# WindowsXp-Beta/nos

Measured on AMD Instinct MI355X. Metric: aggregate GPU util % + schedulable fractional pods/node at 1/2/4/8 MI355X, higher is better.
Workload: dtype fp32

## Files before the change

csrc/hip/gemm_f32h.hip:

```cpp
#include <stdlib.h>

#include <type_traits>

#include "attn_d64_planes.h"
#include "common.h"
#include "epilogue.h"
#include "lds_pipe.h"
#include "split_f16.h"

namespace {

using nos::gelu_erf;
using nos::glds16;
using nos::wait_stages;

template <int E>
using EpiC = std::integral_constant<int, E>;

struct Batch {
  int nb = 1;
  long long a = 0, rinv = 0, w = 0, csc = 0, c = 0, r = 0, bias = 0;
};

constexpr int BK = 32;

__device__ __forceinline__ int swz(int row) { return (row >> 2) & 3; }

using nos::kvp::KvOut;

struct PlaneOut {
  unsigned short* p = nullptr;
  long long pplane = 0;
  int ldp = 0;
  float sc = 1.f;
};

struct LnIo {
  const float* x = nullptr;
  const float2* sin = nullptr;
  float2* sout = nullptr;
  int ldx = 0, nparts = 0, pw = 0, spart = 0;
  float eps = 0.f, sc = 1.f;
};

__device__ __forceinline__ void chan_merge(float& n, float& mean, float& m2, float nb, float mb, float m2b) {
  const float tot = n + nb;
  if (!(nb > 0.f)) return;
  const float d = mb - mean, f = nb / tot;
  mean = fmaf(d, f, mean);
  m2 += m2b + d * d * n * f;
  n = tot;
}

template <int BM, int BN, int WGM, int WGN, bool PERSIST, int RS = 2, int MODE = 0, bool BATCHED = false>
__global__ __launch_bounds__(64 * WGM * WGN, 2) void gemm_h3_kernel(
    const _Float16* __restrict__ Ap, int lda, long long aplane, const float* __restrict__ rinv, float rconst,
    const _Float16* __restrict__ Wp, int ldw, long long wplane, const float* __restrict__ csc,
    const float* __restrict__ bias, const float* __restrict__ R, int ldr0, float* __restrict__ C, int ldc0, int M,
    int N, int K, int epi, int tiles_m, int tiles_n, KvOut kv, PlaneOut po, Batch bt, LnIo ln) {
  constexpr int NW = WGM * WGN, MI = BM / (32 * WGM), NI = BN / (32 * WGN);
  static_assert(NW == 4 && MI >= 1 && NI >= 1, "4 waves");
  constexpr int ROWB = BK * 2, CH = ROWB / 16, RPP = 1024 / ROWB;
  static_assert(RS == 2 || RS == 3, "ring depth");
  constexpr int TA = 2 * BM * ROWB, STAGE = TA + 2 * BN * ROWB;
  constexpr int APW = TA / 1024 / NW, WPW = 2 * BN * ROWB / 1024 / NW;
  static_assert(APW * NW * 1024 == TA && WPW * NW * 1024 == 2 * BN * ROWB, "equal DMA count per wave");
  constexpr int LPS = APW + WPW;
  static_assert((RS - 2) * LPS < 64, "vmcnt range");
  static_assert(MODE == 0 || (BM == 128 && !BATCHED && (BN == 128 || BN == 64) && (RS == 2 || (MODE == 2 && RS == 3))),
                "the LayerNorm hand-off runs 128 x 128 or 128 x 64 tiles (the producer also on a 3-deep ring)");
  static_assert(MODE != 2 || BM * BN * 4 <= RS * STAGE, "the statistics tile fits the ring");
  extern __shared__ __attribute__((aligned(16))) unsigned char smem[];

  const int tid = threadIdx.x, wid = __builtin_amdgcn_readfirstlane(tid >> 6), lane = tid & 63;
  const int c0 = lane & 31, h0 = lane >> 5;
  const int wm = wid / WGN, wn = wid % WGN;
  const bool wide = (epi & EPI_WIDE) != 0;
  epi &= ~EPI_WIDE;
  const int ntiles1 = tiles_m * tiles_n, ntiles = BATCHED ? ntiles1 * bt.nb : ntiles1;
  const int nk = K / BK;
  nos::XcdChunk chunk;
  if constexpr (PERSIST) {
    chunk = nos::xcd_chunk(blockIdx.x, gridDim.x, ntiles);
  } else {
    chunk.first = nos::xcd_remap(blockIdx.x, ntiles);
    chunk.end = chunk.first + 1;
    chunk.step = 1;
  }
  for (int tt = chunk.first; tt < chunk.end; tt += chunk.step) {
    if (PERSIST && tt != chunk.first) __syncthreads();
    const int bb = BATCHED ? tt / ntiles1 : 0, t1 = BATCHED ? tt - bb * ntiles1 : tt;
    const int tm = t1 / tiles_n, tn = t1 - tm * tiles_n;
    const int m0 = tm * BM, n0 = tn * BN;
    const _Float16* __restrict__ Ab = BATCHED ? Ap + bb * bt.a : Ap;
    const _Float16* __restrict__ Wb = BATCHED ? Wp + bb * bt.w : Wp;
    const float* __restrict__ rinvb = BATCHED && rinv != nullptr ? rinv + bb * bt.rinv : rinv;
    const float* __restrict__ cscb = BATCHED ? csc + bb * bt.csc : csc;
    float* __restrict__ Cb = BATCHED && C != nullptr ? C + bb * bt.c : C;
// ... 9 lines not shown
        int g = m0 + row;
        g = g < M ? g : M - 1;
        glds16(Ab + plane * aplane + (long long)g * lda + k0 + (((lane % CH) ^ swz(row)) << 3),
               dst + plane * BM * ROWB + rb * ROWB);
      }
    };
    auto stage_w = [&](int k0, unsigned char* dst) {
#pragma unroll
      for (int i = 0; i < WPW; ++i) {
        const int p = wid * WPW + i;
        const int plane = p / (BN / RPP), rb = (p % (BN / RPP)) * RPP;
        const int row = rb + lane / CH;
        int g = n0 + row;
        g = g < N ? g : N - 1;
        glds16(Wb + plane * wplane + (long long)g * ldw + k0 + (((lane % CH) ^ swz(row)) << 3),
               dst + TA + plane * BN * ROWB + rb * ROWB);
      }
    };
    auto stage = [&](int k0, unsigned char* dst) {
      stage_a(k0, dst);
      stage_w(k0, dst);
    };

    f32x16_t acc[MI][NI];
#pragma unroll
    for (int i = 0; i < MI; ++i)
#pragma unroll
      for (int j = 0; j < NI; ++j)
#pragma unroll
        for (int r = 0; r < 16; ++r) acc[i][j][r] = 0.f;

    struct Frag {
      f16x8_t a[MI][2], w[NI][2];
    };
    auto load = [&](const unsigned char* base, int s, Frag& f) {
#pragma unroll
      for (int i = 0; i < MI; ++i) {
        const int row = wm * (BM / WGM) + i * 32 + c0;
#pragma unroll
        for (int p = 0; p < 2; ++p)
          f.a[i][p] = *reinterpret_cast<const f16x8_t*>(base + p * BM * ROWB + row * ROWB +
                                                        (((2 * s + h0) ^ swz(row)) << 4));
      }
#pragma unroll
      for (int j = 0; j < NI; ++j) {
        const int row = wn * (BN / WGN) + j * 32 + c0;
#pragma unroll
        for (int p = 0; p < 2; ++p)
          f.w[j][p] = *reinterpret_cast<const f16x8_t*>(base + TA + p * BN * ROWB + row * ROWB +
                                                        (((2 * s + h0) ^ swz(row)) << 4));
      }
    };
    auto mma = [&](const Frag& f) {
#pragma unroll
      for (int i = 0; i < MI; ++i)
#pragma unroll
        for (int j = 0; j < NI; ++j) acc[i][j] = nos::mma3h(f.a[i], f.w[j], acc[i][j]);
    };

    if constexpr (MODE == 1) {
    constexpr int AR = BM * 4 / (64 * NW);
    constexpr int RSTEP = 64 * NW / 4;
    const int q = tid & 3;
    float mul[AR], add[AR];
    const float* xr[AR];
#pragma unroll
    for (int i = 0; i < AR; ++i) {
      int g = m0 + (tid >> 2) + RSTEP * i;
      g = g < M ? g : M - 1;
      xr[i] = ln.x + (long long)g * ln.ldx + q * 8;
      const float2* st = ln.sin + (long long)g * ln.nparts;
      float n = 0.f, mean = 0.f, m2 = 0.f;
      for (int p = 0; p < ln.nparts; ++p) {
        const float2 v = st[p];
        const int nb = min(ln.pw, K - p * ln.pw);
        chan_merge(n, mean, m2, (float)nb, v.x, v.y);
      }
      mul[i] = rsqrtf(m2 / (float)K + ln.eps) * ln.sc;
      add[i] = -mean * mul[i];
    }
    float4 xa[AR][2];
// ... 9 lines not shown
      for (int i = 0; i < AR; ++i) {
        const int row = (tid >> 2) + RSTEP * i;
        const float4 u = xa[i][0], w = xa[i][1];
        f16x2_t h0, l0, h1, l1, h2, l2, h3, l3;
        nos::split2h(f32x2_t{fmaf(u.x, mul[i], add[i]), fmaf(u.y, mul[i], add[i])}, h0, l0);
        nos::split2h(f32x2_t{fmaf(u.z, mul[i], add[i]), fmaf(u.w, mul[i], add[i])}, h1, l1);
        nos::split2h(f32x2_t{fmaf(w.x, mul[i], add[i]), fmaf(w.y, mul[i], add[i])}, h2, l2);
        nos::split2h(f32x2_t{fmaf(w.z, mul[i], add[i]), fmaf(w.w, mul[i], add[i])}, h3, l3);
        const int off = row * ROWB + ((q ^ swz(row)) << 4);
        *reinterpret_cast<f16x8_t*>(dst + off) = f16x8_t{h0.x, h0.y, h1.x, h1.y, h2.x, h2.y, h3.x, h3.y};
        *reinterpret_cast<f16x8_t*>(dst + BM * ROWB + off) = f16x8_t{l0.x, l0.y, l1.x, l1.y, l2.x, l2.y, l3.x, l3.y};
      }
    };
    aload(0);
    stage_w(0, smem);
    asm volatile("s_waitcnt vmcnt(0)" ::: "memory");
    awrite(smem);
    if (nk > 1) {
      aload(BK);
      stage_w(BK, smem + STAGE);
    }
    asm volatile("s_waitcnt lgkmcnt(0)" ::: "memory");
    __builtin_amdgcn_s_barrier();
    Frag fa, fb;
    load(smem, 0, fa);
    for (int kt = 0; kt < nk; ++kt) {
      const unsigned char* cur = smem + (kt & 1) * STAGE;
      load(cur, 1, fb);
      mma(fa);
      __builtin_amdgcn_sched_barrier(0);
      if (kt + 1 < nk) {
        asm volatile("s_waitcnt vmcnt(0)" ::: "memory");
        awrite(smem + ((kt + 1) & 1) * STAGE);
      }
      __builtin_amdgcn_sched_barrier(0);
      mma(fb);
      __builtin_amdgcn_sched_barrier(0);
      if (kt + 1 < nk) {
        asm volatile("s_waitcnt lgkmcnt(0)" ::: "memory");
        __builtin_amdgcn_s_barrier();
        if (kt + 2 < nk) {
          aload((kt + 2) * BK);
          stage_w((kt + 2) * BK, smem + (kt & 1) * STAGE);
        }
        load(smem + ((kt + 1) & 1) * STAGE, 0, fa);
      }
      __builtin_amdgcn_sched_barrier(0);
    }
    } else if constexpr (RS == 2) {
    stage(0, smem);
    if (nk > 1) stage(BK, smem + STAGE);
    if (nk > 1) {
      asm volatile("s_waitcnt vmcnt(%0)" ::"n"(LPS) : "memory");
    } else {
      asm volatile("s_waitcnt vmcnt(0)" ::: "memory");
    }
    __builtin_amdgcn_s_barrier();
    Frag fa, fb;
    load(smem, 0, fa);
    for (int kt = 0; kt < nk; ++kt) {
      const unsigned char* cur = smem + (kt & 1) * STAGE;
      load(cur, 1, fb);
      mma(fa);
      __builtin_amdgcn_sched_barrier(0);
      if (kt + 1 < nk) {
        asm volatile("s_waitcnt vmcnt(0)" ::: "memory");
        asm volatile("s_waitcnt lgkmcnt(0)" ::: "memory");
        __builtin_amdgcn_s_barrier();
        if (kt + 2 < nk) stage((kt + 2) * BK, smem + (kt & 1) * STAGE);
        load(smem + ((kt + 1) & 1) * STAGE, 0, fa);
      }
      mma(fb);
      __builtin_amdgcn_sched_barrier(0);
    }
    } else {
#pragma unroll
    for (int q = 0; q < RS - 1; ++q)
      if (q < nk) stage(q * BK, smem + q * STAGE);
    for (int kt = 0; kt < nk; ++kt) {
      wait_stages<LPS>(min(RS - 2, nk - 1 - kt));
      asm volatile("s_waitcnt lgkmcnt(0)" ::: "memory");
      __builtin_amdgcn_s_barrier();
      if (kt + RS - 1 < nk) stage((kt + RS - 1) * BK, smem + ((kt + RS - 1) % RS) * STAGE);
      const unsigned char* cur = smem + (kt % RS) * STAGE;
      Frag f0, f1;
      load(cur, 0, f0);
      load(cur, 1, f1);
      mma(f0);
      mma(f1);
    }
    }
    __syncthreads();

    int c = c0, h = h0, ldc = ldc0, ldr = ldr0;
    asm volatile("" : "+v"(c), "+v"(h));
    asm volatile("" : "+s"(ldc), "+s"(ldr));
    float rsv[MI][16], rbv[MI][16];
    if (rinvb != nullptr) {
#pragma unroll
      for (int i = 0; i < MI; ++i)
#pragma unroll
        for (int r = 0; r < 16; ++r) {
          const int m = m0 + wm * (BM / WGM) + i * 32 + (r & 3) + 8 * (r >> 2) + 4 * h;
          rsv[i][r] = rinvb[m < M ? m : M - 1];
        }
    } else {
#pragma unroll
      for (int i = 0; i < MI; ++i)
#pragma unroll
        for (int r = 0; r < 16; ++r) rsv[i][r] = rconst;
    }
#pragma unroll
    for (int i = 0; i < MI; ++i)
#pragma unroll
      for (int r = 0; r < 16; ++r) {
        const int m = m0 + wm * (BM / WGM) + i * 32 + (r & 3) + 8 * (r >> 2) + 4 * h;
        rbv[i][r] = (BATCHED && (epi & EPI_BIAS_ROW)) ? biasb[m < M ? m : M - 1] : 0.f;
      }
    auto epilogue = [&](auto ec) -> bool {
      constexpr int E = decltype(ec)::value;
      auto has = [&](int f) -> bool {
        if constexpr (E < 0) return (epi & f) != 0;
        else return (E & f) != 0;
      };
      if constexpr (MODE == 2) {
        float* const T = reinterpret_cast<float*>(smem);
  #pragma unroll
        for (int j = 0; j < NI; ++j) {
          const int cl = wn * (BN / WGN) + j * 32 + c;
          const int nc = n0 + cl < N ? n0 + cl : N - 1;
          const float cs = cscb[nc];
          const float p2 = has(EPI_BIAS) ? biasb[nc] : 0.f;
  #pragma unroll
          for (int i = 0; i < MI; ++i) {
  #pragma unroll
            for (int r = 0; r < 16; ++r) {
              const int rl = wm * (BM / WGM) + i * 32 + (r & 3) + 8 * (r >> 2) + 4 * h;
              float v = fmaf(acc[i][j][r], rsv[i][r] * cs, p2);
              if (has(EPI_GELU)) v = gelu_erf(v);
              if (has(EPI_RELU)) v = fmaxf(v, 0.f);
              T[rl * BN + cl] = v;
            }
          }
        }
        __syncthreads();
        const int rr = tid >> 1, hf = tid & 1, m = m0 + rr;
        const int nv = m < M ? max(0, min(BN / 2, N - n0 - hf * (BN / 2))) : 0;
        const float* tr = T + rr * BN + hf * (BN / 2);
        const long long col0 = n0 + hf * (BN / 2);
        constexpr int HV = BN / 8;
        float4 v[HV];
        const bool want = ln.sout != nullptr;
        float sum = 0.f;
        auto pass1 = [&](auto wholec) {
          constexpr bool W = decltype(wholec)::value;
  #pragma unroll
          for (int u = 0; u < HV; ++u) {
            const int k = ((u + tid) & (HV - 1)) * 4;
            v[u] = *reinterpret_cast<const float4*>(tr + k);
            if (W || k < nv) {
// ... 33 lines not shown
      }
      const bool full = m0 + BM <= M && n0 + BN <= N;
      if (full && !(has(EPI_RESID) || has(EPI_RESID_PRE)) &&
          (po.p != nullptr || (kv.kvs != nullptr && kv.S == M && n0 >= kv.qcols && kv.hd % BN == 0))) {
        unsigned short* hi;
        long long lo_off;
        int ld;
        int t = 0;
        if (po.p != nullptr) {
          hi = po.p + (long long)m0 * po.ldp + n0;
          lo_off = po.pplane;
          ld = po.ldp;
        } else {
          t = (n0 - kv.qcols) >= kv.hd;
          hi = kv.kvs + ((long long)m0 * nos::kvp::H3 + nos::kvp::H3 / 2 * t) * kv.hd + (n0 - kv.qcols - t * kv.hd);
          lo_off = kv.hd;
          ld = nos::kvp::H3 * kv.hd;
        }
        constexpr bool WIDE_FITS = 4 * BM * BN <= RS * STAGE && !BATCHED && (BN == 128 || BN == 64);
        constexpr int SWM = BN / 8 - 1;
        unsigned short* const T = reinterpret_cast<unsigned short*>(smem);
  #pragma unroll
        for (int j = 0; j < NI; ++j) {
          const int cl = wn * (BN / WGN) + j * 32 + c;
          const float cs = cscb[n0 + cl];
          const float p2 = has(EPI_BIAS) ? biasb[n0 + cl] : 0.f;
          const float osc = po.p != nullptr ? po.sc : kv.kvsc[t * (kv.hd >> 6) + ((n0 - kv.qcols - t * kv.hd + cl) >> 6)];
  #pragma unroll
          for (int i = 0; i < MI; ++i) {
  #pragma unroll
            for (int r = 0; r < 16; ++r) {
              const int rl = wm * (BM / WGM) + i * 32 + (r & 3) + 8 * (r >> 2) + 4 * h;
              float v = fmaf(acc[i][j][r], rsv[i][r] * cs, p2 + rbv[i][r]);
              if (has(EPI_GELU)) v = gelu_erf(v);
              if (has(EPI_RELU)) v = fmaxf(v, 0.f);
              const float x = v * osc;
              const _Float16 h0 = (_Float16)x;
              const _Float16 h1 = (_Float16)(x - (float)h0);
              if (WIDE_FITS && wide) {
                const int sl = rl * BN + ((((cl >> 3) ^ (rl & SWM)) << 3) | (cl & 7));
                T[sl] = __builtin_bit_cast(unsigned short, h0);
                T[BM * BN + sl] = __builtin_bit_cast(unsigned short, h1);
              } else {
                const unsigned off = (unsigned)(rl * ld + cl);
                hi[off] = __builtin_bit_cast(unsigned short, h0);
                hi[lo_off + off] = __builtin_bit_cast(unsigned short, h1);
              }
            }
          }
        }
        if (WIDE_FITS && wide) {
          __syncthreads();
          constexpr int CPR = BN / 8;
          constexpr int NCH = 2 * BM * CPR;
  #pragma unroll
          for (int q = 0; q < NCH / (64 * NW); ++q) {
            const int id = tid + q * 64 * NW;
            const int pl = id / (BM * CPR), rem = id - pl * (BM * CPR);
            const int row = rem / CPR, ch = rem - row * CPR;
            const uint4 v = *reinterpret_cast<const uint4*>(T + pl * BM * BN + row * BN + ((ch ^ (row & SWM)) << 3));
            *reinterpret_cast<uint4*>(hi + pl * lo_off + (long long)row * ld + ch * 8) = v;
          }
        }
        return true;
      }
      const bool interior = full && po.p == nullptr && (kv.kvs == nullptr || n0 + BN <= kv.qcols);
      if (interior) {
        float* Ct = Cb + (long long)m0 * ldc + n0;
        const float* Rt = has(EPI_RESID) || (BATCHED && has(EPI_RESID_PRE)) ? Rb + (long long)m0 * ldr + n0 : nullptr;
  #pragma unroll
        for (int j = 0; j < NI; ++j) {
          const int cl = wn * (BN / WGN) + j * 32 + c;
          const float cs = cscb[n0 + cl];
          const float p2 = has(EPI_BIAS) ? biasb[n0 + cl] : 0.f;
  #pragma unroll
          for (int i = 0; i < MI; ++i) {
  #pragma unroll
            for (int r = 0; r < 16; ++r) {
              const int rl = wm * (BM / WGM) + i * 32 + (r & 3) + 8 * (r >> 2) + 4 * h;
              float v = fmaf(acc[i][j][r], rsv[i][r] * cs, p2 + rbv[i][r]);
              if (BATCHED && has(EPI_RESID_PRE)) v += Rt[(unsigned)(rl * ldr + cl)];
              if (has(EPI_GELU)) v = gelu_erf(v);
              if (has(EPI_RELU)) v = fmaxf(v, 0.f);
              if (has(EPI_RESID)) v += Rt[(unsigned)(rl * ldr + cl)];
              Ct[(unsigned)(rl * ldc + cl)] = v;
            }
          }
        }
        return true;
      }
      return false;
    };
    bool done = false;
    if constexpr (MODE == 1) {
      if (epi == EPI_BIAS) done = epilogue(EpiC<EPI_BIAS>{});
      else if (epi == (EPI_BIAS | EPI_GELU)) done = epilogue(EpiC<EPI_BIAS | EPI_GELU>{});
      else done = epilogue(EpiC<-1>{});
    } else if constexpr (MODE == 2) {
      if (epi == (EPI_BIAS | EPI_RESID)) done = epilogue(EpiC<EPI_BIAS | EPI_RESID>{});
      else if (epi == EPI_BIAS) done = epilogue(EpiC<EPI_BIAS>{});
      else done = epilogue(EpiC<-1>{});
    } else if constexpr (BATCHED) {
      done = epilogue(EpiC<-1>{});
    } else {
      switch (epi) {
        case EPI_BIAS: done = epilogue(EpiC<EPI_BIAS>{}); break;
        case EPI_BIAS | EPI_GELU: done = epilogue(EpiC<EPI_BIAS | EPI_GELU>{}); break;
        case EPI_BIAS | EPI_RESID: done = epilogue(EpiC<EPI_BIAS | EPI_RESID>{}); break;
        default: done = epilogue(EpiC<-1>{}); break;
      }
    }
    if (done) continue;
#pragma unroll
    for (int j = 0; j < NI; ++j) {
      const int n = n0 + wn * (BN / WGN) + j * 32 + c;
      const int nc = n < N ? n : N - 1;
      const float cs = cscb[nc];
      const float p2 = (epi & EPI_BIAS) ? biasb[nc] : 0.f;
#pragma unroll
      for (int i = 0; i < MI; ++i) {
#pragma unroll
        for (int r = 0; r < 16; ++r) {
          const int m = m0 + wm * (BM / WGM) + i * 32 + (r & 3) + 8 * (r >> 2) + 4 * h;
          float v = fmaf(acc[i][j][r], rsv[i][r] * cs, p2 + rbv[i][r]);
          if (BATCHED && (epi & EPI_RESID_PRE) && m < M && n < N) v += Rb[(long long)m * ldr + n];
          if ((epi & EPI_GELU)) v = gelu_erf(v);
          if ((epi & EPI_RELU)) v = fmaxf(v, 0.f);
          if (m < M && n < N) {
            if ((epi & EPI_RESID)) v += Rb[(long long)m * ldr + n];
            if (kv.kvs != nullptr && n >= kv.qcols) {
              const int t = (n - kv.qcols) >= kv.hd;
              const int col = n - kv.qcols - t * kv.hd;
              const int b = kv.S == M ? 0 : m / kv.S;
              const long long row = (long long)b * kv.skvp + (m - b * kv.S);
              const float x = v * kv.kvsc[t * (kv.hd >> 6) + (col >> 6)];
              const _Float16 h0 = (_Float16)x;
              const _Float16 h1 = (_Float16)(x - (float)h0);
              unsigned short* dst = kv.kvs + (row * nos::kvp::H3 + nos::kvp::H3 / 2 * t) * kv.hd + col;
              dst[0] = __builtin_bit_cast(unsigned short, h0);
              dst[kv.hd] = __builtin_bit_cast(unsigned short, h1);
            } else if (po.p != nullptr) {
              const float x = v * po.sc;
              const _Float16 h0 = (_Float16)x;
              const _Float16 h1 = (_Float16)(x - (float)h0);
              po.p[(long long)m * po.ldp + n] = __builtin_bit_cast(unsigned short, h0);
              po.p[po.pplane + (long long)m * po.ldp + n] = __builtin_bit_cast(unsigned short, h1);
// ... 468 lines not shown
```

csrc/hip/probes.hip:

```cpp
#include "common.h"

NOS_API int nos_gemm_bf16(const void* A, int lda, const void* W, int ldw, const void* bias,
                          const void* R, int ldr, void* C, int ldc, int M, int N, int K, int epi,
                          int max_wg, hipStream_t stream);

namespace {

__global__ void probe_placement_kernel(uint4* __restrict__ out, int spin) {
  unsigned xcc, hwid;
  asm volatile("s_getreg_b32 %0, hwreg(HW_REG_XCC_ID)" : "=s"(xcc));
  asm volatile("s_getreg_b32 %0, hwreg(HW_REG_HW_ID)" : "=s"(hwid));
  const unsigned long long t0 = __builtin_amdgcn_s_memrealtime();
  unsigned long long t = t0;
  while ((int)(t - t0) < spin) t = __builtin_amdgcn_s_memrealtime();
  if (threadIdx.x == 0) out[blockIdx.x] = make_uint4(xcc, hwid, blockIdx.x, (unsigned)t0);
}

__global__ __launch_bounds__(256) void probe_hbm_copy_kernel(const uint4* __restrict__ src,
                                                            uint4* __restrict__ dst, long long n) {
  const long long stride = (long long)gridDim.x * blockDim.x;
  long long i = (long long)blockIdx.x * blockDim.x + threadIdx.x;
  for (; i + 3 * stride < n; i += 4 * stride) {
    const uint4 a = src[i], b = src[i + stride], c = src[i + 2 * stride], d = src[i + 3 * stride];
    dst[i] = a;
// ... 39 lines not shown
__global__ __launch_bounds__(256) void probe_mfma_peak_kernel(float* __restrict__ out, int iters,
                                                              unsigned seed) {
  const int lane = threadIdx.x & 63;
  s16x8_t a16, b16;
#pragma unroll
  for (int j = 0; j < 8; ++j) {
    unsigned x = (seed ^ (lane * 2654435761u) ^ (j * 40503u)) * 2246822519u;
    a16[j] = (short)(0x3c00 | (x & 0x80ff));
    b16[j] = (short)(0x3c00 | ((x >> 16) & 0x80ff));
  }
  const bf16x8_t a = __builtin_bit_cast(bf16x8_t, a16);
  const bf16x8_t b = __builtin_bit_cast(bf16x8_t, b16);
  f32x16_t c0 = {}, c1 = {}, c2 = {}, c3 = {};
  for (int i = 0; i < iters; ++i) {
    c0 = __builtin_amdgcn_mfma_f32_32x32x16_bf16(a, b, c0, 0, 0, 0);
    c1 = __builtin_amdgcn_mfma_f32_32x32x16_bf16(a, b, c1, 0, 0, 0);
    c2 = __builtin_amdgcn_mfma_f32_32x32x16_bf16(a, b, c2, 0, 0, 0);
    c3 = __builtin_amdgcn_mfma_f32_32x32x16_bf16(a, b, c3, 0, 0, 0);
  }
  float s = 0.f;
#pragma unroll
  for (int i = 0; i < 16; ++i) s += c0[i] + c1[i] + c2[i] + c3[i];
  if (s == 1234.5f) out[blockIdx.x] = s;
}

struct EventTimer {
  hipEvent_t a = nullptr, b = nullptr;
  EventTimer() { (void)hipEventCreate(&a); (void)hipEventCreate(&b); }
  ~EventTimer() { (void)hipEventDestroy(a); (void)hipEventDestroy(b); }
};

}

NOS_API int nos_probe_placement(void* out_dev, int nwg, int spin_ticks, hipStream_t stream) {
  if (nwg <= 0) return (int)hipErrorInvalidValue;
  hipLaunchKernelGGL(probe_placement_kernel, dim3(nwg), dim3(64), 0, stream, (uint4*)out_dev,
                     spin_ticks);
  return (int)hipGetLastError();
}

NOS_API int nos_probe_hbm_copy(const void* src, void* dst, long long bytes, int nwg,
                               hipStream_t stream) {
  if (bytes <= 0 || (bytes % 16) || nwg <= 0) return (int)hipErrorInvalidValue;
  hipLaunchKernelGGL(probe_hbm_copy_kernel, dim3(nwg), dim3(256), 0, stream, (const uint4*)src,
                     (uint4*)dst, bytes / 16);
  return (int)hipGetLastError();
// ... 46 lines not shown
  (void)hipEventElapsedTime(&ms, tm.a, tm.b);
  const double moved = (mode == 2 ? 1.0 : 2.0) * (double)bytes * iters;
  *gbps = (ms > 0.f) ? moved / (ms * 1e-3) / 1e9 : 0.0;
  (void)hipFree(src);
  (void)hipFree(dst);
  return rc;
}

NOS_API int nos_probe_mfma_peak(hipStream_t stream, int nwg, int iters, double* tflops) {
  float* scratch = nullptr;
  HIP_CHECK_RET(hipMalloc(&scratch, sizeof(float) * nwg));
  hipLaunchKernelGGL(probe_mfma_peak_kernel, dim3(nwg), dim3(256), 0, stream, scratch, 64, 7u);
  EventTimer tm;
  (void)hipEventRecord(tm.a, stream);
  hipLaunchKernelGGL(probe_mfma_peak_kernel, dim3(nwg), dim3(256), 0, stream, scratch, iters, 11u);
  (void)hipEventRecord(tm.b, stream);
  (void)hipEventSynchronize(tm.b);
  int rc = (int)hipGetLastError();
  float ms = 0.f;
  (void)hipEventElapsedTime(&ms, tm.a, tm.b);
  const double flop = (double)nwg * 4  * iters * 4  * (32.0 * 32 * 16 * 2);
  *tflops = (ms > 0.f) ? flop / (ms * 1e-3) / 1e12 : 0.0;
  (void)hipFree(scratch);
  return rc;
}

NOS_API int nos_probe_mfma_peak_launch(hipStream_t stream, int nwg, int iters, void* scratch) {
  if (nwg <= 0 || iters <= 0) return (int)hipErrorInvalidValue;
  hipLaunchKernelGGL(probe_mfma_peak_kernel, dim3(nwg), dim3(256), 0, stream, (float*)scratch, iters, 13u);
  return (int)hipGetLastError();
}

NOS_API int nos_probe_gemm(hipStream_t stream, int n, int iters, int max_wg, double* tflops) {
  if (n <= 0 || (n % 128)) return (int)hipErrorInvalidValue;
  const size_t bytes = (size_t)n * n * 2;
  void *a = nullptr, *w = nullptr, *c = nullptr;
  HIP_CHECK_RET(hipMalloc(&a, bytes));
  HIP_CHECK_RET(hipMalloc(&w, bytes));
  HIP_CHECK_RET(hipMalloc(&c, bytes));
  (void)hipMemsetAsync(a, 0x3c, bytes, stream);
  (void)hipMemsetAsync(w, 0x3c, bytes, stream);
  int rc = nos_gemm_bf16(a, n, w, n, nullptr, nullptr, 0, c, n, n, n, n, 0, max_wg, stream);
  EventTimer tm;
  (void)hipEventRecord(tm.a, stream);
  for (int i = 0; i < iters && rc == 0; ++i)
    rc = nos_gemm_bf16(a, n, w, n, nullptr, nullptr, 0, c, n, n, n, n, 0, max_wg, stream);
// ... 11 lines not shown
```

csrc/hip/split_f16.h:

```cpp
#pragma once
#include "common.h"

typedef __attribute__((ext_vector_type(8))) _Float16 f16x8_t;
typedef __attribute__((ext_vector_type(2))) _Float16 f16x2_t;

namespace nos {

__device__ __forceinline__ void split2h(f32x2_t x, f16x2_t& hi, f16x2_t& lo) {
  hi = __builtin_convertvector(x, f16x2_t);
  const unsigned hb = __builtin_bit_cast(unsigned, hi);
  unsigned lb;
  asm("v_fma_mixlo_f16 %0, %1, 1.0, -%2 op_sel_hi:[0,0,1]\n\t"
      "v_fma_mixhi_f16 %0, %3, 1.0, -%2 op_sel:[0,0,1] op_sel_hi:[0,0,1]"
      : "=&v"(lb)
      : "v"(x.x), "v"(hb), "v"(x.y));
  lo = __builtin_bit_cast(f16x2_t, lb);
}

__device__ __forceinline__ void split8h(const float (&x)[8], float sc, f16x8_t& hi, f16x8_t& lo) {
#pragma unroll
  for (int j = 0; j < 8; j += 2) {
    f16x2_t h2, l2;
    split2h(f32x2_t{x[j] * sc, x[j + 1] * sc}, h2, l2);
    hi[j] = h2.x; hi[j + 1] = h2.y;
// ... 3 lines not shown

__device__ __forceinline__ void set_pair(f16x8_t (&f)[2][2], int j2, f32x2_t v) {
  f16x2_t hi, lo;
  split2h(v, hi, lo);
  const int s2 = j2 >> 2, e = 2 * (j2 & 3);
  f[s2][0][e] = hi.x; f[s2][0][e + 1] = hi.y;
  f[s2][1][e] = lo.x; f[s2][1][e + 1] = lo.y;
}

__device__ __forceinline__ void store_acc32(float* p, const f32x16_t& acc, float f, int hh) {
#pragma unroll
  for (int g = 0; g < 4; ++g)
    *reinterpret_cast<float4*>(p + 8 * g + 4 * hh) =
        float4{acc[4 * g] * f, acc[4 * g + 1] * f, acc[4 * g + 2] * f, acc[4 * g + 3] * f};
}

__device__ __forceinline__ f32x16_t mma3h(const f16x8_t (&a)[2], const f16x8_t (&b)[2], f32x16_t acc) {
  acc = __builtin_amdgcn_mfma_f32_32x32x16_f16(a[1], b[0], acc, 0, 0, 0);
  acc = __builtin_amdgcn_mfma_f32_32x32x16_f16(a[0], b[1], acc, 0, 0, 0);
  acc = __builtin_amdgcn_mfma_f32_32x32x16_f16(a[0], b[0], acc, 0, 0, 0);
  return acc;
}

__device__ __forceinline__ float pow2i(int e) { return __int_as_float((e + 127) << 23); }

__device__ __forceinline__ int h3_scale_exp(float vmax) {
  if (!(vmax > 0.f)) return 0;
  int e;
  frexpf(vmax, &e);
  e = 14 - e;
  return e < -126 ? -126 : (e > 126 ? 126 : e);
}

}
```

nos_amd/ops/_lib.py:

```python
from __future__ import annotations

import ctypes
import os
import threading
from pathlib import Path

_LIB_PATH = Path(os.environ.get("NOS_AMD_HIP_LIB") or
                 Path(__file__).resolve().parent.parent / "_native" / "libnos_hip.so")
_lock = threading.Lock()
_lib: ctypes.CDLL | None = None
_err: str | None = None

c_int, c_ll, c_float, c_void_p, c_double = (ctypes.c_int, ctypes.c_longlong, ctypes.c_float,
                                            ctypes.c_void_p, ctypes.c_double)

_SIGS = {
    "nos_attn_fwd_d64": [c_void_p, c_void_p, c_void_p, c_void_p, c_int, c_int, c_int, c_int, c_int,
                         c_ll, c_int, c_ll, c_float, c_void_p],
    "nos_attn_fwd_f32_d64": [c_void_p, c_void_p, c_void_p, c_void_p, c_int, c_int, c_int, c_int, c_int,
                             c_ll, c_int, c_ll, c_float, c_void_p],
    "nos_attn_fwd_f32x6_d64": [c_void_p, c_void_p, c_void_p, c_void_p, c_int, c_int, c_int, c_int, c_int,
                               c_ll, c_int, c_ll, c_float, c_void_p, c_ll, c_void_p],
    "nos_attn_f32x6_workspace": [c_int, c_int, c_int, c_int],
    "nos_attn_fwd_f32x6_presplit_d64": [c_void_p, c_void_p, c_int, c_int, c_int, c_int, c_int, c_ll, c_int, c_ll,
# ... 20 lines not shown
                        c_int, c_float, c_void_p],
    "nos_gemm_f32x6": [c_void_p, c_int, c_void_p, c_int, c_ll, c_void_p, c_void_p, c_int, c_void_p, c_int, c_int,
                       c_int, c_int, c_int, c_void_p],
    "nos_gemm_ln_f32x6": [c_void_p, c_int, c_void_p, c_int, c_ll, c_void_p, c_void_p, c_void_p, c_int, c_int, c_int,
                          c_int, c_int, c_float, c_void_p],
    "nos_gemm_f32_pick_tile": [c_int, c_int],
    "nos_gemm_f32x6_set_stage": [c_int],
    "nos_gemm_f32x6_set_tile": [c_int],
    "nos_gemm_f32x6_set_pipeline": [c_int],
    "nos_gemm_set_policy": [c_int],
    "nos_gemm_set_persistent": [c_int],
    "nos_gemm_f32_set_policy": [c_int],
    "nos_attn_f32_set_variant": [c_int],
    "nos_gemm_ln_bf16": [c_void_p, c_int, c_void_p, c_int, c_void_p, c_void_p, c_void_p, c_int, c_int, c_int,
                         c_int, c_int, c_float, c_int, c_void_p],
    "nos_layernorm_bf16": [c_void_p, c_void_p, c_void_p, c_void_p, c_void_p, c_void_p, c_int, c_int,
                           c_int, c_int, c_int, c_int, c_float, c_void_p],
    "nos_probe_placement": [c_void_p, c_int, c_int, c_void_p],
    "nos_probe_hbm_copy": [c_void_p, c_void_p, c_ll, c_int, c_void_p],
    "nos_probe_hbm": [c_void_p, c_ll, c_int, c_int, ctypes.POINTER(c_double)],
    "nos_probe_hbm_mode": [c_void_p, c_ll, c_int, c_int, c_int, ctypes.POINTER(c_double)],
    "nos_probe_mfma_peak": [c_void_p, c_int, c_int, ctypes.POINTER(c_double)],
    "nos_probe_mfma_peak_launch": [c_void_p, c_int, c_int, c_void_p],
    "nos_probe_gemm": [c_void_p, c_int, c_int, c_int, ctypes.POINTER(c_double)],
    "nos_stream_create_cumask": [ctypes.POINTER(ctypes.c_uint), c_int, ctypes.POINTER(c_void_p)],
    "nos_stream_get_cumask": [c_void_p, c_int, ctypes.POINTER(ctypes.c_uint)],
    "nos_stream_destroy": [c_void_p],
    "nos_stream_sync": [c_void_p],
    "nos_device_info": [c_int, ctypes.POINTER(c_int), ctypes.POINTER(c_ll), ctypes.POINTER(c_int),
                        ctypes.c_char_p, c_int],
    "nos_runtime_version": [ctypes.POINTER(c_int)],
    "nos_set_cu_budget": [c_int],
    "nos_get_cu_budget": [],
    "nos_gemm_f32h3_batched": [c_void_p, c_int, c_ll, c_ll, c_void_p, c_ll, c_float, c_void_p, c_int, c_ll, c_ll,
                               c_void_p, c_ll, c_void_p, c_ll, c_void_p, c_int, c_ll, c_void_p, c_int, c_ll, c_int,
                               c_int, c_int, c_int, c_int, c_void_p],
    "nos_embedding": [c_void_p, c_void_p, c_void_p, c_ll, c_int, c_int, c_void_p],
    "nos_rmsnorm": [c_void_p, c_void_p, c_void_p, c_int, c_int, c_int, c_int, c_float, c_int, c_void_p],
    "nos_softmax": [c_void_p, c_void_p, c_int, c_int, c_int, c_int, c_int, c_void_p],
    "nos_rotary": [c_void_p, c_void_p, c_void_p, c_void_p, c_int, c_int, c_int, c_int, c_int, c_ll, c_int, c_void_p],
    "nos_im2col_h3": [c_void_p, c_void_p, c_ll, c_void_p, c_int, c_int, c_int, c_int, c_int, c_int, c_int, c_int,
                      c_int, c_int, c_int, c_int, c_int, c_void_p],
    "nos_im2col": [c_void_p, c_ll, c_ll, c_ll, c_void_p, c_ll, c_void_p, c_int, c_int, c_int, c_int, c_int, c_int,
                   c_int, c_int, c_int, c_int, c_int, c_int, c_int, c_int, c_void_p],
    "nos_unary": [c_void_p, c_int, c_void_p, c_int, c_ll, c_int, c_void_p],
    "nos_unary_rows": [c_void_p, c_ll, c_int, c_void_p, c_int, c_ll, c_int, c_int, c_void_p],
# ... 128 lines not shown
```

nos_amd/ops/probes.py:

```python
from __future__ import annotations

import ctypes
from collections import Counter
from dataclasses import dataclass

import torch

from . import _lib


@dataclass
class Placement:
    xcc: int
    se: int
    sh: int
    cu: int
    block: int

    @property
    def cu_key(self) -> tuple[int, int, int, int]:
        return (self.xcc, self.se, self.sh, self.cu)


def decode_hw_id(hw_id: int) -> tuple[int, int, int]:
# ... 22 lines not shown

def hbm_gbps(stream: int, bytes_: int = 1 << 30, iters: int = 5, nwg: int = 2048) -> float:
    v = ctypes.c_double()
    _lib.check(_lib.lib().nos_probe_hbm(stream, bytes_, iters, nwg, ctypes.byref(v)), "probe_hbm")
    return v.value


HBM_MODES = {"copy": 0, "copy_nt": 1, "read": 2}


def hbm_mode_gbps(stream: int, mode: str = "copy_nt", bytes_: int = 1 << 30, iters: int = 5, nwg: int = 2048) -> float:
    v = ctypes.c_double()
    _lib.check(_lib.lib().nos_probe_hbm_mode(stream, bytes_, iters, nwg, HBM_MODES[mode], ctypes.byref(v)),
               "probe_hbm_mode")
    return v.value


def mfma_peak_tflops(stream: int, nwg: int, iters: int = 20000) -> float:
    v = ctypes.c_double()
    _lib.check(_lib.lib().nos_probe_mfma_peak(stream, nwg, iters, ctypes.byref(v)), "probe_mfma_peak")
    return v.value


def gemm_tflops(stream: int, n: int = 4096, iters: int = 5, max_wg: int = 0) -> float:
    v = ctypes.c_double()
    _lib.check(_lib.lib().nos_probe_gemm(stream, n, iters, max_wg, ctypes.byref(v)), "probe_gemm")
    return v.value
```

Before: 28.00.

## Switch split-f16 GEMM to 16x16x32 MFMA with half-fragment software pipeline

Result: no change. 28.00 (+0.0%).

```diff
diff --git a/csrc/hip/gemm_f32h.hip b/csrc/hip/gemm_f32h.hip
--- a/csrc/hip/gemm_f32h.hip
+++ b/csrc/hip/gemm_f32h.hip
@@ -24,7 +24,10 @@
 
 constexpr int BK = 32;
 
-__device__ __forceinline__ int swz(int row) { return (row >> 2) & 3; }
+__device__ __forceinline__ int swz(int row) { return -(row >> 2) & 3; }
+
+__device__ __forceinline__ int acc_row(int i, int g, int r) { return 16 * i + 4 * g + r; }
+__device__ __forceinline__ int acc_col(int j, int c) { return 16 * j + c; }
 
 using nos::kvp::KvOut;
 
@@ -58,8 +61,9 @@
     const _Float16* __restrict__ Wp, int ldw, long long wplane, const float* __restrict__ csc,
     const float* __restrict__ bias, const float* __restrict__ R, int ldr0, float* __restrict__ C, int ldc0, int M,
     int N, int K, int epi, int tiles_m, int tiles_n, KvOut kv, PlaneOut po, Batch bt, LnIo ln) {
-  constexpr int NW = WGM * WGN, MI = BM / (32 * WGM), NI = BN / (32 * WGN);
-  static_assert(NW == 4 && MI >= 1 && NI >= 1, "4 waves");
+  constexpr int NW = WGM * WGN, MI = BM / (16 * WGM), NI = BN / (16 * WGN);
+  constexpr int AH = MI / 2, WH = NI / 2;
+  static_assert(NW == 4 && AH >= 1 && WH >= 1 && 2 * AH == MI && 2 * WH == NI, "4 waves, two halves each way");
   constexpr int ROWB = BK * 2, CH = ROWB / 16, RPP = 1024 / ROWB;
   static_assert(RS == 2 || RS == 3, "ring depth");
   constexpr int TA = 2 * BM * ROWB, STAGE = TA + 2 * BN * ROWB;
@@ -73,7 +77,7 @@
   extern __shared__ __attribute__((aligned(16))) unsigned char smem[];
 
   const int tid = threadIdx.x, wid = __builtin_amdgcn_readfirstlane(tid >> 6), lane = tid & 63;
-  const int c0 = lane & 31, h0 = lane >> 5;
+  const int c0 = lane & 15, g0 = lane >> 4;
   const int wm = wid / WGN, wn = wid % WGN;
   const bool wide = (epi & EPI_WIDE) != 0;
   epi &= ~EPI_WIDE;
@@ -129,41 +133,51 @@
       stage_w(k0, dst);
     };
 
-    f32x16_t acc[MI][NI];
+    f32x4_t acc[MI][NI];
 #pragma unroll
     for (int i = 0; i < MI; ++i)
 #pragma unroll
       for (int j = 0; j < NI; ++j)
 #pragma unroll
-        for (int r = 0; r < 16; ++r) acc[i][j][r] = 0.f;
-
-    struct Frag {
-      f16x8_t a[MI][2], w[NI][2];
-    };
-    auto load = [&](const unsigned char* base, int s, Frag& f) {
-#pragma unroll
-      for (int i = 0; i < MI; ++i) {
-        const int row = wm * (BM / WGM) + i * 32 + c0;
+        for (int r = 0; r < 4; ++r) acc[i][j][r] = 0.f;
+
+    struct FragA {
+      f16x8_t a[AH][2];
+    };
+    struct FragW {
+      f16x8_t w[WH][2];
+    };
+    FragA fa[2];
+    FragW fw[2];
+    auto load_a = [&](const unsigned char* base, int h, FragA& f) {
+#pragma unroll
+      for (int i = 0; i < AH; ++i) {
+        const int row = wm * (BM / WGM) + (h * AH + i) * 16 + c0;
 #pragma unroll
         for (int p = 0; p < 2; ++p)
-          f.a[i][p] = *reinterpret_cast<const f16x8_t*>(base + p * BM * ROWB + row * ROWB +
-                                                        (((2 * s + h0) ^ swz(row)) << 4));
-      }
-#pragma unroll
-      for (int j = 0; j < NI; ++j) {
-        const int row = wn * (BN / WGN) + j * 32 + c0;
+          f.a[i][p] = *reinterpret_cast<const f16x8_t*>(base + p * BM * ROWB + row * ROWB + ((g0 ^ swz(row)) << 4));
+      }
+    };
+    auto load_w = [&](const unsigned char* base, int h, FragW& f) {
+#pragma unroll
+      for (int j = 0; j < WH; ++j) {
+        const int row = wn * (BN / WGN) + (h * WH + j) * 16 + c0;
 #pragma unroll
         for (int p = 0; p < 2; ++p)
-          f.w[j][p] = *reinterpret_cast<const f16x8_t*>(base + TA + p * BN * ROWB + row * ROWB +
-                                                        (((2 * s + h0) ^ swz(row)) << 4));
-      }
-    };
-    auto mma = [&](const Frag& f) {
-#pragma unroll
-      for (int i = 0; i < MI; ++i)
-#pragma unroll
-        for (int j = 0; j < NI; ++j) acc[i][j] = nos::mma3h(f.a[i], f.w[j], acc[i][j]);
-    };
+          f.w[j][p] =
+              *reinterpret_cast<const f16x8_t*>(base + TA + p * BN * ROWB + row * ROWB + ((g0 ^ swz(row)) << 4));
+      }
+    };
+    auto mma = [&](auto hac, auto hwc) {
+      constexpr int HA = decltype(hac)::value, HW = decltype(hwc)::value;
+#pragma unroll
+      for (int i = 0; i < AH; ++i)
+#pragma unroll
+        for (int j = 0; j < WH; ++j)
+          acc[HA * AH + i][HW * WH + j] = nos::mma3h16(fa[HA].a[i], fw[HW].w[j], acc[HA * AH + i][HW * WH + j]);
+    };
+    using H0 = std::integral_constant<int, 0>;
+    using H1 = std::integral_constant<int, 1>;
 
     if constexpr (MODE == 1) {
     constexpr int AR = BM * 4 / (64 * NW);
@@ -219,19 +233,24 @@
     }
     asm volatile("s_waitcnt lgkmcnt(0)" ::: "memory");
     __builtin_amdgcn_s_barrier();
-    Frag fa, fb;
-    load(smem, 0, fa);
-    for (int kt = 0; kt < nk; ++kt) {
+    load_a(smem, 0, fa[0]);
+    load_w(smem, 0, fw[0]);
+    auto kstep = [&](int kt, auto fc) {
+      using F = decltype(fc);
+      using S = std::integral_constant<int, 1 - F::value>;
       const unsigned char* cur = smem + (kt & 1) * STAGE;
-      load(cur, 1, fb);
-      mma(fa);
+      load_w(cur, S::value, fw[S::value]);
+      load_a(cur, 1, fa[1]);
+      mma(H0{}, F{});
+      mma(H0{}, S{});
       __builtin_amdgcn_sched_barrier(0);
       if (kt + 1 < nk) {
         asm volatile("s_waitcnt vmcnt(0)" ::: "memory");
         awrite(smem + ((kt + 1) & 1) * STAGE);
       }
       __builtin_amdgcn_sched_barrier(0);
-      mma(fb);
+      mma(H1{}, S{});
+      mma(H1{}, F{});
       __builtin_amdgcn_sched_barrier(0);
       if (kt + 1 < nk) {
         asm volatile("s_waitcnt lgkmcnt(0)" ::: "memory");
@@ -240,9 +259,14 @@
           aload((kt + 2) * BK);
           stage_w((kt + 2) * BK, smem + (kt & 1) * STAGE);
         }
-        load(smem + ((kt + 1) & 1) * STAGE, 0, fa);
+        load_a(smem + ((kt + 1) & 1) * STAGE, 0, fa[0]);
+        load_w(smem + ((kt + 1) & 1) * STAGE, S::value, fw[S::value]);
       }
       __builtin_amdgcn_sched_barrier(0);
+    };
+    for (int kt = 0; kt < nk; kt += 2) {
+      kstep(kt, H0{});
+      if (kt + 1 < nk) kstep(kt + 1, H1{});
     }
     } else if constexpr (RS == 2) {
     stage(0, smem);
@@ -253,22 +277,35 @@
       asm volatile("s_waitcnt vmcnt(0)" ::: "memory");
     }
     __builtin_amdgcn_s_barrier();
-    Frag fa, fb;
-    load(smem, 0, fa);
-    for (int kt = 0; kt < nk; ++kt) {
+    load_a(smem, 0, fa[0]);
+    load_w(smem, 0, fw[0]);
+    auto kstep = [&](int kt, auto fc) {
+      using F = decltype(fc);
+      using S = std::integral_constant<int, 1 - F::value>;
       const unsigned char* cur = smem + (kt & 1) * STAGE;
-      load(cur, 1, fb);
-      mma(fa);
+      const unsigned char* nxt = smem + ((kt + 1) & 1) * STAGE;
+      load_w(cur, S::value, fw[S::value]);
+      mma(H0{}, F{});
+      __builtin_amdgcn_sched_barrier(0);
+      load_a(cur, 1, fa[1]);
+      mma(H0{}, S{});
       __builtin_amdgcn_sched_barrier(0);
       if (kt + 1 < nk) {
         asm volatile("s_waitcnt vmcnt(0)" ::: "memory");
         asm volatile("s_waitcnt lgkmcnt(0)" ::: "memory");
         __builtin_amdgcn_s_barrier();
         if (kt + 2 < nk) stage((kt + 2) * BK, smem + (kt & 1) * STAGE);
-        load(smem + ((kt + 1) & 1) * STAGE, 0, fa);
-      }
-      mma(fb);
+        load_a(nxt, 0, fa[0]);
+      }
+      mma(H1{}, S{});
       __builtin_amdgcn_sched_barrier(0);
+      if (kt + 1 < nk) load_w(nxt, S::value, fw[S::value]);
+      mma(H1{}, F{});
+      __builtin_amdgcn_sched_barrier(0);
+    };
+    for (int kt = 0; kt < nk; kt += 2) {
+      kstep(kt, H0{});
+      if (kt + 1 < nk) kstep(kt + 1, H1{});
     }
     } else {
 #pragma unroll
@@ -280,38 +317,41 @@
       __builtin_amdgcn_s_barrier();
       if (kt + RS - 1 < nk) stage((kt + RS - 1) * BK, smem + ((kt + RS - 1) % RS) * STAGE);
       const unsigned char* cur = smem + (kt % RS) * STAGE;
-      Frag f0, f1;
-      load(cur, 0, f0);
-      load(cur, 1, f1);
-      mma(f0);
-      mma(f1);
+      load_a(cur, 0, fa[0]);
+      load_w(cur, 0, fw[0]);
+      load_w(cur, 1, fw[1]);
+      load_a(cur, 1, fa[1]);
+      mma(H0{}, H0{});
+      mma(H0{}, H1{});
+      mma(H1{}, H1{});
+      mma(H1{}, H0{});
     }
     }
     __syncthreads();
 
-    int c = c0, h = h0, ldc = ldc0, ldr = ldr0;
-    asm volatile("" : "+v"(c), "+v"(h));
+    int c = c0, g = g0, ldc = ldc0, ldr = ldr0;
+    asm volatile("" : "+v"(c), "+v"(g));
     asm volatile("" : "+s"(ldc), "+s"(ldr));
-    float rsv[MI][16], rbv[MI][16];
+    float rsv[MI][4], rbv[MI][4];
     if (rinvb != nullptr) {
 #pragma unroll
       for (int i = 0; i < MI; ++i)
 #pragma unroll
-        for (int r = 0; r < 16; ++r) {
-          const int m = m0 + wm * (BM / WGM) + i * 32 + (r & 3) + 8 * (r >> 2) + 4 * h;
+        for (int r = 0; r < 4; ++r) {
+          const int m = m0 + wm * (BM / WGM) + acc_row(i, g, r);
           rsv[i][r] = rinvb[m < M ? m : M - 1];
         }
     } else {
 #pragma unroll
       for (int i = 0; i < MI; ++i)
 #pragma unroll
-        for (int r = 0; r < 16; ++r) rsv[i][r] = rconst;
+        for (int r = 0; r < 4; ++r) rsv[i][r] = rconst;
     }
 #pragma unroll
     for (int i = 0; i < MI; ++i)
 #pragma unroll
-      for (int r = 0; r < 16; ++r) {
-        const int m = m0 + wm * (BM / WGM) + i * 32 + (r & 3) + 8 * (r >> 2) + 4 * h;
+      for (int r = 0; r < 4; ++r) {
+        const int m = m0 + wm * (BM / WGM) + acc_row(i, g, r);
         rbv[i][r] = (BATCHED && (epi & EPI_BIAS_ROW)) ? biasb[m < M ? m : M - 1] : 0.f;
       }
     auto epilogue = [&](auto ec) -> bool {
@@ -324,15 +364,15 @@
         float* const T = reinterpret_cast<float*>(smem);
   #pragma unroll
         for (int j = 0; j < NI; ++j) {
-          const int cl = wn * (BN / WGN) + j * 32 + c;
+          const int cl = wn * (BN / WGN) + acc_col(j, c);
           const int nc = n0 + cl < N ? n0 + cl : N - 1;
           const float cs = cscb[nc];
           const float p2 = has(EPI_BIAS) ? biasb[nc] : 0.f;
   #pragma unroll
           for (int i = 0; i < MI; ++i) {
   #pragma unroll
-            for (int r = 0; r < 16; ++r) {
-              const int rl = wm * (BM / WGM) + i * 32 + (r & 3) + 8 * (r >> 2) + 4 * h;
+            for (int r = 0; r < 4; ++r) {
+              const int rl = wm * (BM / WGM) + acc_row(i, g, r);
               float v = fmaf(acc[i][j][r], rsv[i][r] * cs, p2);
               if (has(EPI_GELU)) v = gelu_erf(v);
               if (has(EPI_RELU)) v = fmaxf(v, 0.f);
@@ -412,15 +452,15 @@
         unsigned short* const T = reinterpret_cast<unsigned short*>(smem);
   #pragma unroll
         for (int j = 0; j < NI; ++j) {
-          const int cl = wn * (BN / WGN) + j * 32 + c;
+          const int cl = wn * (BN / WGN) + acc_col(j, c);
           const float cs = cscb[n0 + cl];
           const float p2 = has(EPI_BIAS) ? biasb[n0 + cl] : 0.f;
           const float osc = po.p != nullptr ? po.sc : kv.kvsc[t * (kv.hd >> 6) + ((n0 - kv.qcols - t * kv.hd + cl) >> 6)];
   #pragma unroll
           for (int i = 0; i < MI; ++i) {
   #pragma unroll
-            for (int r = 0; r < 16; ++r) {
-              const int rl = wm * (BM / WGM) + i * 32 + (r & 3) + 8 * (r >> 2) + 4 * h;
+            for (int r = 0; r < 4; ++r) {
+              const int rl = wm * (BM / WGM) + acc_row(i, g, r);
               float v = fmaf(acc[i][j][r], rsv[i][r] * cs, p2 + rbv[i][r]);
               if (has(EPI_GELU)) v = gelu_erf(v);
               if (has(EPI_RELU)) v = fmaxf(v, 0.f);
@@ -460,14 +500,14 @@
         const float* Rt = has(EPI_RESID) || (BATCHED && has(EPI_RESID_PRE)) ? Rb + (long long)m0 * ldr + n0 : nullptr;
   #pragma unroll
         for (int j = 0; j < NI; ++j) {
-          const int cl = wn * (BN / WGN) + j * 32 + c;
+          const int cl = wn * (BN / WGN) + acc_col(j, c);
           const float cs = cscb[n0 + cl];
           const float p2 = has(EPI_BIAS) ? biasb[n0 + cl] : 0.f;
   #pragma unroll
           for (int i = 0; i < MI; ++i) {
   #pragma unroll
-            for (int r = 0; r < 16; ++r) {
-              const int rl = wm * (BM / WGM) + i * 32 + (r & 3) + 8 * (r >> 2) + 4 * h;
+            for (int r = 0; r < 4; ++r) {
+              const int rl = wm * (BM / WGM) + acc_row(i, g, r);
               float v = fmaf(acc[i][j][r], rsv[i][r] * cs, p2 + rbv[i][r]);
               if (BATCHED && has(EPI_RESID_PRE)) v += Rt[(unsigned)(rl * ldr + cl)];
               if (has(EPI_GELU)) v = gelu_erf(v);
@@ -503,15 +543,15 @@
     if (done) continue;
 #pragma unroll
     for (int j = 0; j < NI; ++j) {
-      const int n = n0 + wn * (BN / WGN) + j * 32 + c;
+      const int n = n0 + wn * (BN / WGN) + acc_col(j, c);
       const int nc = n < N ? n : N - 1;
       const float cs = cscb[nc];
       const float p2 = (epi & EPI_BIAS) ? biasb[nc] : 0.f;
 #pragma unroll
       for (int i = 0; i < MI; ++i) {
 #pragma unroll
-        for (int r = 0; r < 16; ++r) {
-          const int m = m0 + wm * (BM / WGM) + i * 32 + (r & 3) + 8 * (r >> 2) + 4 * h;
+        for (int r = 0; r < 4; ++r) {
+          const int m = m0 + wm * (BM / WGM) + acc_row(i, g, r);
           float v = fmaf(acc[i][j][r], rsv[i][r] * cs, p2 + rbv[i][r]);
           if (BATCHED && (epi & EPI_RESID_PRE) && m < M && n < N) v += Rb[(long long)m * ldr + n];
           if ((epi & EPI_GELU)) v = gelu_erf(v);
diff --git a/csrc/hip/probes.hip b/csrc/hip/probes.hip
--- a/csrc/hip/probes.hip
+++ b/csrc/hip/probes.hip
@@ -1,3 +1,9 @@
+#include <math.h>
+
+#include <algorithm>
+#include <type_traits>
+#include <vector>
+
 #include "common.h"
 
 NOS_API int nos_gemm_bf16(const void* A, int lda, const void* W, int ldw, const void* bias,
@@ -85,6 +91,110 @@
 #pragma unroll
   for (int i = 0; i < 16; ++i) s += c0[i] + c1[i] + c2[i] + c3[i];
   if (s == 1234.5f) out[blockIdx.x] = s;
+}
+
+typedef __attribute__((ext_vector_type(8))) _Float16 ph16x8_t;
+
+template <bool S16>
+__global__ __launch_bounds__(256, 2) void probe_mfma_shape_kernel(float* __restrict__ out,
+                                                                 unsigned long long* __restrict__ stamps, int iters,
+                                                                 unsigned seed) {
+  constexpr int ROWB = 64, PLANE = 64 * ROWB;
+  __shared__ __attribute__((aligned(16))) unsigned char lds[4 * 4 * PLANE];
+  const int tid = threadIdx.x, wid = tid >> 6, lane = tid & 63;
+#pragma unroll
+  for (int i = 0; i < 16; ++i) {
+    const int off = (i * 256 + tid) * 16;
+    const unsigned expo = ((off / PLANE) & 1) ? 0x1000u : 0x3c00u;
+    unsigned w[4];
+#pragma unroll
+    for (int j = 0; j < 4; ++j) {
+      unsigned x = (seed ^ ((unsigned)(off + 4 * j) * 2654435761u) ^ (blockIdx.x * 40503u)) * 2246822519u;
+      x ^= x >> 15;
+      w[j] = (x & 0x83ff83ffu) | expo | (expo << 16);
+    }
+    *reinterpret_cast<uint4*>(lds + off) = make_uint4(w[0], w[1], w[2], w[3]);
+  }
+  __syncthreads();
+  const unsigned char* base = lds + wid * 4 * PLANE;
+  constexpr int NF = 16;
+  auto frag_off = [&](int q) -> int {
+    const int op = q >> 3, p = q & 1;
+    int row, ch, sw;
+    if constexpr (S16) {
+      row = ((q >> 1) & 3) * 16 + (lane & 15);
+      ch = lane >> 4;
+      sw = (4 - ((row >> 2) & 3)) & 3;
+    } else {
+      row = ((q >> 1) & 1) * 32 + (lane & 31);
+      ch = 2 * ((q >> 2) & 1) + (lane >> 5);
+      sw = (row >> 2) & 3;
+    }
+    return (2 * op + p) * PLANE + row * ROWB + ((ch ^ sw) << 4);
+  };
+  int offs[NF];
+#pragma unroll
+  for (int q = 0; q < NF; ++q) offs[q] = frag_off(q);
+  using acc_t = std::conditional_t<S16, f32x4_t, f32x16_t>;
+  constexpr int NB = S16 ? 4 : 2;
+  acc_t acc[NB][NB];
+#pragma unroll
+  for (int i = 0; i < NB; ++i)
+#pragma unroll
+    for (int j = 0; j < NB; ++j) acc[i][j] = acc_t{};
+  auto load = [&](ph16x8_t (&f)[NF]) {
+    asm volatile("" ::: "memory");
+#pragma unroll
+    for (int q = 0; q < NF; ++q) f[q] = *reinterpret_cast<const ph16x8_t*>(base + offs[q]);
+  };
+  auto mma = [&](const ph16x8_t (&f)[NF]) {
+    if constexpr (S16) {
+#pragma unroll
+      for (int i = 0; i < 4; ++i)
+#pragma unroll
+        for (int j = 0; j < 4; ++j) {
+          const ph16x8_t ah = f[2 * i], al = f[2 * i + 1], wh = f[8 + 2 * j], wl = f[8 + 2 * j + 1];
+          acc[i][j] = __builtin_amdgcn_mfma_f32_16x16x32_f16(al, wh, acc[i][j], 0, 0, 0);
+          acc[i][j] = __builtin_amdgcn_mfma_f32_16x16x32_f16(ah, wl, acc[i][j], 0, 0, 0);
+          acc[i][j] = __builtin_amdgcn_mfma_f32_16x16x32_f16(ah, wh, acc[i][j], 0, 0, 0);
+        }
+    } else {
+#pragma unroll
+      for (int s = 0; s < 2; ++s)
+#pragma unroll
+        for (int i = 0; i < 2; ++i)
+#pragma unroll
+          for (int j = 0; j < 2; ++j) {
+            const ph16x8_t ah = f[4 * s + 2 * i], al = f[4 * s + 2 * i + 1];
+            const ph16x8_t wh = f[8 + 4 * s + 2 * j], wl = f[8 + 4 * s + 2 * j + 1];
+            acc[i][j] = __builtin_amdgcn_mfma_f32_32x32x16_f16(al, wh, acc[i][j], 0, 0, 0);
+            acc[i][j] = __builtin_amdgcn_mfma_f32_32x32x16_f16(ah, wl, acc[i][j], 0, 0, 0);
+            acc[i][j] = __builtin_amdgcn_mfma_f32_32x32x16_f16(ah, wh, acc[i][j], 0, 0, 0);
+          }
+    }
+  };
+  ph16x8_t fa[NF], fb[NF];
+  load(fa);
+  const unsigned long long c0 = __builtin_amdgcn_s_memtime(), r0 = __builtin_amdgcn_s_memrealtime();
+  for (int it = 0; it < iters; it += 2) {
+    load(fb);
+    mma(fa);
+    load(fa);
+    mma(fb);
+  }
+  const unsigned long long c1 = __builtin_amdgcn_s_memtime(), r1 = __builtin_amdgcn_s_memrealtime();
+  float s = 0.f;
+#pragma unroll
+  for (int i = 0; i < NB; ++i)
+#pragma unroll
+    for (int j = 0; j < NB; ++j)
+#pragma unroll
+      for (int r = 0; r < (S16 ? 4 : 16); ++r) s += acc[i][j][r];
+  if (s == 1234.5f) out[blockIdx.x] = s;
+  if (lane == 0) {
+    stamps[2 * (blockIdx.x * 4 + wid)] = c1 - c0;
+    stamps[2 * (blockIdx.x * 4 + wid) + 1] = r1 - r0;
+  }
 }
 
 struct EventTimer {
@@ -177,6 +287,59 @@
   const double flop = (double)nwg * 4  * iters * 4  * (32.0 * 32 * 16 * 2);
   *tflops = (ms > 0.f) ? flop / (ms * 1e-3) / 1e12 : 0.0;
   (void)hipFree(scratch);
+  return rc;
+}
+
+NOS_API int nos_probe_mfma_shape(hipStream_t stream, int shape, int nwg, int iters, double seconds, double* res) {
+  if (nwg <= 0 || iters <= 0 || (iters & 1) || shape < 0 || shape > 1 || !(seconds >= 0.0)) return (int)hipErrorInvalidValue;
+  float* out = nullptr;
+  unsigned long long* stamps = nullptr;
+  const size_t nst = (size_t)nwg * 4 * 2;
+  HIP_CHECK_RET(hipMalloc(&out, sizeof(float) * nwg));
+  HIP_CHECK_RET(hipMalloc(&stamps, sizeof(unsigned long long) * nst));
+  unsigned seed = 1u;
+  auto launch = [&]() {
+    if (shape == 1)
+      hipLaunchKernelGGL(probe_mfma_shape_kernel<true>, dim3(nwg), dim3(256), 0, stream, out, stamps, iters, seed++);
+    else
+      hipLaunchKernelGGL(probe_mfma_shape_kernel<false>, dim3(nwg), dim3(256), 0, stream, out, stamps, iters, seed++);
+  };
+  auto timed = [&](int n) -> float {
+    EventTimer tm;
+    (void)hipEventRecord(tm.a, stream);
+    for (int i = 0; i < n; ++i) launch();
+    (void)hipEventRecord(tm.b, stream);
+    (void)hipEventSynchronize(tm.b);
+    float ms = 0.f;
+    (void)hipEventElapsedTime(&ms, tm.a, tm.b);
+    return ms;
+  };
+  launch();
+  const float one = timed(1);
+  const int batch = one > 0.f ? (int)fmin(1000.0, fmax(1.0, 250.0 / one)) : 1;
+  double spent = 0.0;
+  while (spent < seconds * 1e3) {
+    const float ms = timed(batch);
+    if (!(ms > 0.f)) break;
+    spent += ms;
+  }
+  const float ms = timed(batch);
+  int rc = (int)hipGetLastError();
+  std::vector<unsigned long long> h(nst);
+  if (rc == 0) rc = (int)hipMemcpy(h.data(), stamps, sizeof(unsigned long long) * nst, hipMemcpyDeviceToHost);
+  std::vector<double> cyc(nst / 2), mhz(nst / 2);
+  for (size_t i = 0; i < nst / 2; ++i) {
+    cyc[i] = (double)h[2 * i] / iters;
+    mhz[i] = h[2 * i + 1] ? 100.0 * (double)h[2 * i] / (double)h[2 * i + 1] : 0.0;
+  }
+  std::nth_element(cyc.begin(), cyc.begin() + cyc.size() / 2, cyc.end());
+  std::nth_element(mhz.begin(), mhz.begin() + mhz.size() / 2, mhz.end());
+  const double flop = (double)nwg * 4  * iters * batch * (64.0 * 64 * 32 * 2 * 3);
+  res[0] = ms > 0.f ? flop / (ms * 1e-3) / 1e12 : 0.0;
+  res[1] = cyc[cyc.size() / 2];
+  res[2] = mhz[mhz.size() / 2];
+  (void)hipFree(out);
+  (void)hipFree(stamps);
   return rc;
 }
 
diff --git a/csrc/hip/split_f16.h b/csrc/hip/split_f16.h
--- a/csrc/hip/split_f16.h
+++ b/csrc/hip/split_f16.h
@@ -49,6 +49,13 @@
   return acc;
 }
 
+__device__ __forceinline__ f32x4_t mma3h16(const f16x8_t (&a)[2], const f16x8_t (&b)[2], f32x4_t acc) {
+  acc = __builtin_amdgcn_mfma_f32_16x16x32_f16(a[1], b[0], acc, 0, 0, 0);
+  acc = __builtin_amdgcn_mfma_f32_16x16x32_f16(a[0], b[1], acc, 0, 0, 0);
+  acc = __builtin_amdgcn_mfma_f32_16x16x32_f16(a[0], b[0], acc, 0, 0, 0);
+  return acc;
+}
+
 __device__ __forceinline__ float pow2i(int e) { return __int_as_float((e + 127) << 23); }
 
 __device__ __forceinline__ int h3_scale_exp(float vmax) {
diff --git a/nos_amd/ops/_lib.py b/nos_amd/ops/_lib.py
--- a/nos_amd/ops/_lib.py
+++ b/nos_amd/ops/_lib.py
@@ -66,6 +66,7 @@
     "nos_probe_hbm_mode": [c_void_p, c_ll, c_int, c_int, c_int, ctypes.POINTER(c_double)],
     "nos_probe_mfma_peak": [c_void_p, c_int, c_int, ctypes.POINTER(c_double)],
     "nos_probe_mfma_peak_launch": [c_void_p, c_int, c_int, c_void_p],
+    "nos_probe_mfma_shape": [c_void_p, c_int, c_int, c_int, c_double, ctypes.POINTER(c_double)],
     "nos_probe_gemm": [c_void_p, c_int, c_int, c_int, ctypes.POINTER(c_double)],
     "nos_stream_create_cumask": [ctypes.POINTER(ctypes.c_uint), c_int, ctypes.POINTER(c_void_p)],
     "nos_stream_get_cumask": [c_void_p, c_int, ctypes.POINTER(ctypes.c_uint)],
diff --git a/nos_amd/ops/probes.py b/nos_amd/ops/probes.py
--- a/nos_amd/ops/probes.py
+++ b/nos_amd/ops/probes.py
@@ -68,6 +68,15 @@
     return v.value
 
 
+MFMA_SHAPES = {"32x32x16": 0, "16x16x32": 1}
+
+
+def mfma_shape(stream: int, shape: str, nwg: int = 512, iters: int = 4000, seconds: float = 2.0) -> dict:
+    res = (ctypes.c_double * 3)()
+    _lib.check(_lib.lib().nos_probe_mfma_shape(stream, MFMA_SHAPES[shape], nwg, iters, seconds, res), "probe_mfma_shape")
+    return {"shape": shape, "tflops": res[0], "wave_cycles_per_stage": res[1], "clock_mhz": res[2]}
+
+
 def gemm_tflops(stream: int, n: int = 4096, iters: int = 5, max_wg: int = 0) -> float:
     v = ctypes.c_double()
     _lib.check(_lib.lib().nos_probe_gemm(stream, n, iters, max_wg, ctypes.byref(v)), "probe_gemm")
```
